# minhtrangvy/distributed_bitcoin_minter

Hardware: AMD Instinct MI355X
Metric: GH/s (SHA-256 "msg nonce" min-search) at 1/2/4/8 MI355X; % of int32 VALU peak (higher is better)
Workload: dtype u32

## Files before the change

### distributed_bitcoin_minter_amd/_lib.py

```python
import ctypes
import os

_HERE = os.path.dirname(os.path.abspath(__file__))
LIB_PATH = os.environ.get("BTCMINER_LIB") or os.path.join(_HERE, "libbtcminer.so")

BM_OK = 0
BM_EINVAL = -1
BM_ENODEV = -2
BM_EHIP = -3
BM_ERCCL = -4
BM_ENOMEM = -5
BM_EINTERNAL = -6
BM_EPEER = -7
BM_ETIMEDOUT = -8
BM_EFULL = -9
BM_MAX_LAUNCH_STATS = 64
BM_MAX_STAT_DEVICES = 16
BM_RCCL_ID_BYTES = 128
BM_ABI_VERSION = 7
BM_DEFAULT_PEER_TIMEOUT_MS = 600_000
BM_COMBINE_AUTO, BM_COMBINE_RCCL, BM_COMBINE_HOST = 0, 1, 2
BM_COMBINED_NONE, BM_COMBINED_RCCL, BM_COMBINED_HOST, BM_COMBINED_LOCAL = 0, 1, 2, 3
COMBINED_NAMES = {0: "none", 1: "rccl", 2: "host", 3: "local"}
U64_MAX = (1 << 64) - 1
# ... 314 lines not shown
                                ctypes.c_size_t, c_u32, c_u32, P(JobVerdict), P(PoolVerifyResult)], ctypes.c_int),
        "bm_jobs_verify_cpu": ([P(PoolJobStruct), ctypes.c_size_t, P(PoolSessionStruct), ctypes.c_size_t, P(JobsSubmit),
                                ctypes.c_size_t, P(JobVerdict), P(PoolVerifyResult)], ctypes.c_int),
        "bm_jobs_verify_gpu": ([vp, P(PoolJobStruct), ctypes.c_size_t, P(PoolSessionStruct), ctypes.c_size_t,
                                P(JobsSubmit), ctypes.c_size_t, P(JobVerdict), P(PoolVerifyResult)], ctypes.c_int),
        "bm_share_set_verify_jobs": ([vp, P(PoolJobStruct), ctypes.c_size_t, P(PoolSessionStruct), ctypes.c_size_t,
                                      P(JobsSubmit), ctypes.c_size_t, P(JobVerdict), P(ShareSetResult)], ctypes.c_int),
        "bm_share_set_create": ([vp, ctypes.c_size_t, P(vp)], ctypes.c_int),
        "bm_share_set_create_cpu": ([ctypes.c_size_t, P(vp)], ctypes.c_int),
        "bm_share_set_destroy": ([vp], None),
        "bm_share_set_clear": ([vp], ctypes.c_int),
        "bm_share_set_count": ([vp, P(c_u64), P(c_u64)], ctypes.c_int),
        "bm_share_set_verify": ([vp, P(JobStruct), P(PoolSessionStruct), ctypes.c_size_t, P(PoolSubmit), ctypes.c_size_t,
                                 c_u32, c_u32, P(JobVerdict), P(ShareSetResult)], ctypes.c_int),
        "bm_ledger_create": ([vp, ctypes.c_size_t, P(vp)], ctypes.c_int),
        "bm_ledger_create_cpu": ([ctypes.c_size_t, P(vp)], ctypes.c_int),
        "bm_ledger_destroy": ([vp], None),
        "bm_ledger_clear": ([vp], ctypes.c_int),
        "bm_ledger_rows": ([vp, P(c_u64)], ctypes.c_int),
        "bm_ledger_read": ([vp, ctypes.c_size_t, ctypes.c_size_t, P(LedgerRow)], ctypes.c_int),
        "bm_ledger_drain": ([vp, ctypes.c_size_t, ctypes.c_size_t, P(LedgerRow)], ctypes.c_int),
        "bm_ledger_set_peel": ([vp, c_u32], ctypes.c_int),
        "bm_ledger_verify_jobs": ([vp, vp, P(PoolJobStruct), ctypes.c_size_t, P(PoolSessionStruct), ctypes.c_size_t,
                                   P(c_u32), P(c_u64), P(JobsSubmit), ctypes.c_size_t, P(JobVerdict),
                                   P(LedgerResult)], ctypes.c_int),
        "bm_hash_gpu": ([vp, ctypes.c_char_p, ctypes.c_size_t, P(c_u64), ctypes.c_size_t, P(c_u64)],
                        ctypes.c_int),
        "bm_ctx_set_timing": ([vp, ctypes.c_int], ctypes.c_int),
        "bm_ctx_last_stats": ([vp, P(Stats)], ctypes.c_int),
        "bm_ctx_set_blocks_per_cu": ([vp, ctypes.c_int], ctypes.c_int),
        "bm_ctx_set_max_windows": ([vp, ctypes.c_int], ctypes.c_int),
        "bm_ctx_set_combine": ([vp, ctypes.c_int], ctypes.c_int),
        "bm_ctx_set_task_digits": ([vp, ctypes.c_int], ctypes.c_int),
        "bm_ctx_set_split": ([vp, P(ctypes.c_uint32), ctypes.c_int], ctypes.c_int),
        "bm_ctx_get_split": ([vp, P(ctypes.c_uint32), ctypes.c_int, P(ctypes.c_int)], ctypes.c_int),
        "bm_ctx_set_balance": ([vp, ctypes.c_int], ctypes.c_int),
        "bm_split_range": ([c_u64, c_u64, P(ctypes.c_uint32), ctypes.c_int, P(c_u64), P(c_u64)], ctypes.c_int),
        "bm_plan_segments": ([ctypes.c_char_p, ctypes.c_size_t, c_u64, c_u64, P(Segment), ctypes.c_int,
                              P(ctypes.c_int)], ctypes.c_int),
        "bm_plan_segments_ex": ([ctypes.c_char_p, ctypes.c_size_t, c_u64, c_u64, ctypes.c_int, P(Segment),
                                 ctypes.c_int, P(ctypes.c_int)], ctypes.c_int),
    }
    for name, (args, res) in sigs.items():
        try:
            fn = getattr(lib, name)
        except AttributeError:
            raise OSError(f"{path}: no {name}; rebuild it") from None
        fn.argtypes = args
        fn.restype = res
    if lib.bm_abi_version() != BM_ABI_VERSION:
        raise OSError(f"{path}: ABI version {lib.bm_abi_version()}, expected {BM_ABI_VERSION}; rebuild it")
    return lib


def strerror(status):
    try:
        return load().bm_strerror(status).decode()
    except OSError:
        return f"status {status}"


def check(status, what):
    if status != BM_OK:
        raise BtcMinerError(status, what)


def device_count():
    n = ctypes.c_int(0)
    check(load().bm_device_count(ctypes.byref(n)), "bm_device_count")
    return n.value


def device_pci_bus_id(device: int) -> str:
    buf = ctypes.create_string_buffer(64)
    check(load().bm_device_pci_bus_id(device, buf, len(buf)), "bm_device_pci_bus_id")
    return buf.value.decode()


DEFAULT_MAX_WINDOWS = 64


def plan_segments(msg: bytes, lower: int, upper: int, max_windows: int = DEFAULT_MAX_WINDOWS):
    lib = load()
    n = ctypes.c_int(0)
    f = lib.bm_plan_segments_ex
    check(f(msg, len(msg), lower, upper, max_windows, None, 0, ctypes.byref(n)), "bm_plan_segments")
    arr = (Segment * max(n.value, 1))()
    check(f(msg, len(msg), lower, upper, max_windows, arr, n.value, ctypes.byref(n)), "bm_plan_segments")
    return list(arr[: n.value])


def split_range(lower: int, upper: int, n: int, shares=None):
    lo, hi = (c_u64 * n)(), (c_u64 * n)()
    sh = (ctypes.c_uint32 * n)(*shares) if shares is not None else None
    check(load().bm_split_range(lower, upper, sh, n, lo, hi), "bm_split_range")
    return [(a, b) if a <= b else None for a, b in zip(lo, hi)]


def bits_to_target(nbits: int) -> int:
    if not 0 <= nbits <= U32_MAX:
        raise ValueError(f"bits must be in 0..2^32-1, got {nbits}")
    buf = (ctypes.c_uint8 * 32)()
    if load().bm_header_target_from_bits(nbits, buf) != BM_OK:
        raise ValueError(f"bits {nbits:#010x} is negative or overflows 256 bits")
    return int.from_bytes(bytes(buf), "big")


def roll_versions(base: int, count: int, mask: int = BIP320_MASK):
    for v, what in ((base, "base"), (mask, "mask")):
        if not isinstance(v, int) or isinstance(v, bool) or not 0 <= v <= U32_MAX:
            raise ValueError(f"{what} must be in 0..2^32-1, got {v!r}")
    if not isinstance(count, int) or isinstance(count, bool) or count < 0:
        raise ValueError(f"count must be a non-negative integer, got {count!r}")
    positions = [b for b in range(32) if mask >> b & 1]
    if count > 1 << len(positions):
        raise ValueError(f"mask {mask:#010x} holds {1 << len(positions)} versions, {count} asked for")
    out = []
    for i in range(count):
        v = base & ~mask
        for k, b in enumerate(positions):
            v |= (i >> k & 1) << b
        out.append(v)
    return out


def difficulty_to_target(difficulty) -> int:
    if isinstance(difficulty, bool) or not isinstance(difficulty, (int, float)):
        raise ValueError(f"difficulty must be a number, got {difficulty!r}")
    try:
# ... 722 lines not shown
            hits = [(int.from_bytes(raw[o:o + 32], "big"), int.from_bytes(raw[o + 32:o + 36], "little"))
                    for o in range(0, len(raw), ctypes.sizeof(HeaderHit))]
        return r.count, hits, (int.from_bytes(bytes(r.hash), "big"), r.nonce)

    def header_hash_many(self, header: bytes, nonces):
        header = _header_bytes(header)
        nonces = list(nonces)
        for v in nonces:
            if not 0 <= v <= U32_MAX:
                raise ValueError(f"a nonce must be in 0..2^32-1, got {v!r}")
        n = len(nonces)
        arr = (c_u32 * max(n, 1))(*nonces)
        out = (ctypes.c_uint8 * (32 * max(n, 1)))()
        check(self._lib.bm_header_hash_gpu(self.handle, header, arr, n, out), "bm_header_hash_gpu")
        raw = bytes(out)
        return [int.from_bytes(raw[32 * i:32 * i + 32], "big") for i in range(n)]

    def hash_many(self, msg: bytes, nonces):
        n = len(nonces)
        arr = (c_u64 * max(n, 1))(*nonces)
        out = (c_u64 * max(n, 1))()
        check(self._lib.bm_hash_gpu(self.handle, msg, len(msg), arr, n, out), "bm_hash_gpu")
        return list(out[:n])

    def set_timing(self, on: bool):
        check(self._lib.bm_ctx_set_timing(self.handle, 1 if on else 0), "bm_ctx_set_timing")

    def set_combine(self, mode: int):
        check(self._lib.bm_ctx_set_combine(self.handle, mode), "bm_ctx_set_combine")

    def set_task_digits(self, digits: int):
        check(self._lib.bm_ctx_set_task_digits(self.handle, digits), "bm_ctx_set_task_digits")

    def set_max_windows(self, n: int):
        check(self._lib.bm_ctx_set_max_windows(self.handle, n), "bm_ctx_set_max_windows")

    def set_blocks_per_cu(self, n: int):
        check(self._lib.bm_ctx_set_blocks_per_cu(self.handle, n), "bm_ctx_set_blocks_per_cu")

    def set_split(self, shares):
        shares = list(shares or [])
        arr = (ctypes.c_uint32 * max(len(shares), 1))(*shares)
        check(self._lib.bm_ctx_set_split(self.handle, arr, len(shares)), "bm_ctx_set_split")

    def get_split(self):
        n = ctypes.c_int(0)
        check(self._lib.bm_ctx_get_split(self.handle, None, 0, ctypes.byref(n)), "bm_ctx_get_split")
        arr = (ctypes.c_uint32 * max(n.value, 1))()
        check(self._lib.bm_ctx_get_split(self.handle, arr, n.value, ctypes.byref(n)), "bm_ctx_get_split")
        return list(arr[: n.value])

    def set_balance(self, on: bool):
        check(self._lib.bm_ctx_set_balance(self.handle, 1 if on else 0), "bm_ctx_set_balance")

    def last_stats(self):
        s = Stats()
        check(self._lib.bm_ctx_last_stats(self.handle, ctypes.byref(s)), "bm_ctx_last_stats")
        return s
```

### distributed_bitcoin_minter_amd/csrc/bm_ctx.cpp

```cpp
#include <algorithm>
#include <cerrno>
#include <cstdarg>
#include <cstdio>
#include <cstdlib>
#include <cstring>
#include <system_error>

#include "bm_runtime.hpp"

namespace bm {

void trace(const char* fmt, ...) {
    static const bool on = std::getenv("BTCMINER_TRACE") != nullptr;
    if (!on) return;
    va_list ap;
    va_start(ap, fmt);
    std::fprintf(stderr, "[btcminer] ");
    std::vfprintf(stderr, fmt, ap);
    std::fprintf(stderr, "\n");
    va_end(ap);
}

bool SubmitPool::run(int n, const std::function<void(int)>& f) {
    if (!ensure(n - 1)) return false;
// ... 119 lines not shown
    for (auto& e : d.ev) BM_TRY(new_event(d, e));
    for (auto& s : d.aux) BM_TRY(new_stream(d, s));
    BM_TRY(new_event(d, d.fork, hipEventDisableTiming));
    for (auto& e : d.join) BM_TRY(new_event(d, e, hipEventDisableTiming));
    for (auto& e : d.bal) BM_TRY(new_event(d, e));
    for (auto& e : d.ag) BM_TRY(new_event(d, e));
    BM_TRY(new_event(d, d.own_done, hipEventDisableTiming));
    BM_TRY(ensure_counters(d, kMinCounterStrips));
    return grow(d, d.d_part, d.part_cap, kMinPartials);
}

void destroy_device(DeviceCtx& d) {
    if (d.id < 0) return;
    (void)hipSetDevice(d.id);
    for (hipStream_t s : d.streams) (void)hipStreamSynchronize(s);
    if (d.comm) (void)ncclCommAbort(d.comm);
    d.comm = nullptr;
    for (hipEvent_t e : d.events) (void)hipEventDestroy(e);
    for (const auto& m : d.owned) (void)(m.second ? hipHostFree(m.first) : hipFree(m.first));
    for (hipStream_t s : d.streams) (void)hipStreamDestroy(s);
}

void read_env(bm_ctx* ctx) {
    if (const char* e = std::getenv("BTCMINER_STREAMS")) {
        const int v = std::atoi(e);
        if (v >= 1 && v <= kMaxStreams) ctx->streams = v;
    }
    if (const char* e = std::getenv("BTCMINER_TAIL")) {
        char* end = nullptr;
        errno = 0;
        const unsigned long long v = std::strtoull(e, &end, 10);
        if (end != e && *end == '\0' && errno == 0 && v <= kMaxTailNonces) ctx->tail_nonces = v;
    }
    if (const char* e = std::getenv("BTCMINER_PADC")) ctx->padc = std::strcmp(e, "0") != 0;
    if (const char* e = std::getenv("BTCMINER_HEADER_GROUP")) {
        const int v = std::atoi(e);
        if (v == 1 || v == 2 || v == 4) ctx->header_group = v;
    }
    if (const char* e = std::getenv("BTCMINER_CHUNK")) {
        char* end = nullptr;
        errno = 0;
        const unsigned long long v = std::strtoull(e, &end, 10);
        if (end != e && *end == '\0' && errno == 0 && v >= 10 && v <= 100000) ctx->lane_chunk = v;
    }
}

int create_ctx(const int* devices, int n, int nslots, bm_ctx** out) {
    int count = 0;
    if (hipGetDeviceCount(&count) != hipSuccess || count < 1) return BM_ENODEV;
    for (int i = 0; i < n; ++i)
        if (devices[i] < 0 || devices[i] >= count) return BM_ENODEV;
    bm_ctx* ctx = new (std::nothrow) bm_ctx();
    if (!ctx) return BM_ENOMEM;
    std::memset(&ctx->stats, 0, sizeof ctx->stats);
    std::memset(&ctx->tstats, 0, sizeof ctx->tstats);
    record_rccl(ctx, false);
    read_env(ctx);
    DeviceGuard guard;
    ctx->devs.resize(n);
    for (int i = 0; i < n; ++i) {
        int rc = init_device(ctx->devs[i], devices[i], nslots);
        if (rc != BM_OK) {
            for (auto& d : ctx->devs) destroy_device(d);
            delete ctx;
            return rc;
        }
// ... 265 lines not shown
}

int bm_ctx_set_test_rccl_fault(bm_ctx_t* ctx, int where) {
    if (!ctx || where < 0 || where > 3) return BM_EINVAL;
    ctx->test_rccl_fault = where;
    return BM_OK;
}

int bm_ctx_set_timing(bm_ctx_t* ctx, int enable) {
    if (!ctx) return BM_EINVAL;
    ctx->timing = enable != 0;
    return BM_OK;
}

int bm_ctx_set_blocks_per_cu(bm_ctx_t* ctx, int blocks_per_cu) {
    if (!ctx || blocks_per_cu < 0 || blocks_per_cu > 32) return BM_EINVAL;
    ctx->blocks_per_cu = blocks_per_cu;
    return BM_OK;
}

int bm_ctx_set_combine(bm_ctx_t* ctx, int mode) {
    if (!ctx || mode < BM_COMBINE_AUTO || mode > BM_COMBINE_HOST) return BM_EINVAL;
    if (ctx->rank_ctx && mode != BM_COMBINE_AUTO) return BM_EINVAL;
    ctx->combine = mode;
    return BM_OK;
}

int bm_ctx_set_task_digits(bm_ctx_t* ctx, int digits) {
    if (!ctx || digits < 0 || digits > bm::kMaxInnerDigits) return BM_EINVAL;
    ctx->task_digits = digits;
    return BM_OK;
}

int bm_ctx_set_max_windows(bm_ctx_t* ctx, int max_windows) {
    if (!ctx || max_windows < 0) return BM_EINVAL;
    ctx->max_windows = max_windows;
    return BM_OK;
}

int bm_ctx_set_split(bm_ctx_t* ctx, const uint32_t* shares, int n) {
    if (!ctx || n < 0 || (n > 0 && !shares)) return BM_EINVAL;
    if (n == 0) {
        ctx->shares.clear();
        return BM_OK;
    }
    const int slots = ctx->rank_ctx ? ctx->world : (int)ctx->devs.size();
    if (n != slots) return BM_EINVAL;
    for (int i = 0; i < n; ++i)
        if (shares[i] == 0) return BM_EINVAL;
    ctx->shares.assign(shares, shares + n);
    return BM_OK;
}

int bm_ctx_get_split(const bm_ctx_t* ctx, uint32_t* shares, int cap, int* n) {
    if (!ctx || !n || cap < 0 || (cap > 0 && !shares)) return BM_EINVAL;
    *n = (int)ctx->shares.size();
    for (int i = 0; i < cap && i < *n; ++i) shares[i] = ctx->shares[(size_t)i];
    return BM_OK;
}

int bm_ctx_set_balance(bm_ctx_t* ctx, int enable) {
    if (!ctx || (ctx->rank_ctx && ctx->world > 1 && enable)) return BM_EINVAL;
    ctx->balance = enable != 0;
    return BM_OK;
}

// ... 34 lines not shown
```

### distributed_bitcoin_minter_amd/csrc/bm_plan.cpp

```cpp
#include "bm_plan.hpp"

#include <algorithm>
#include <cstring>

#include "bm_sha256.hpp"

namespace bm {

const uint64_t kPow10[20] = {1ull,
                             10ull,
                             100ull,
                             1000ull,
                             10000ull,
                             100000ull,
                             1000000ull,
                             10000000ull,
                             100000000ull,
                             1000000000ull,
                             10000000000ull,
                             100000000000ull,
                             1000000000000ull,
                             10000000000000ull,
                             100000000000000ull,
                             1000000000000000ull,
// ... 135 lines not shown

std::vector<Piece> slot_pieces(uint64_t lower, uint64_t upper, int n, const std::vector<uint32_t>& shares) {
    const Piece empty{1, 0};
    if (n < 1) return {};
    if (shares.size() != (size_t)n || lower > upper) {
        std::vector<Piece> out = split_range(lower, upper, n);
        out.resize((size_t)n, empty);
        return out;
    }
    std::vector<Piece> out((size_t)n, empty);
    unsigned __int128 total = 0;
    for (int i = 0; i < n; ++i) total += shares[(size_t)i];
    const unsigned __int128 count = (unsigned __int128)(upper - lower) + 1;
    unsigned __int128 prefix = 0, b0 = 0;
    for (int i = 0; i < n; ++i) {
        prefix += shares[(size_t)i];
        const unsigned __int128 b1 = (i == n - 1) ? count : count * prefix / total;
        if (b1 > b0) out[(size_t)i] = Piece{lower + (uint64_t)b0, lower + (uint64_t)(b1 - 1)};
        b0 = b1;
    }
    return out;
}

LaunchGeometry launch_geometry(uint64_t tasks, uint64_t task_nonces, uint64_t lane_chunk, uint64_t resident,
                               uint32_t block) {
    const uint64_t m_max = std::max<uint64_t>(1, lane_chunk / task_nonces);
    const uint64_t m = std::max<uint64_t>(1, std::min<uint64_t>(m_max, tasks / (8 * resident * (uint64_t)block)));
    const uint64_t chunks = (tasks + 64 * m - 1) / (64 * m);
    const uint64_t grid = std::max<uint64_t>(1, std::min<uint64_t>((chunks + 3) / 4, resident));
    const uint64_t k = (chunks + grid * 4 - 1) / (grid * 4);
    return LaunchGeometry{(uint32_t)m, chunks, (uint32_t)grid, k * m};
}

}
```

### distributed_bitcoin_minter_amd/csrc/bm_plan.hpp

```cpp
#pragma once
#include <cstddef>
#include <cstdint>
#include <vector>

#include "btcminer.h"

namespace bm {

extern const uint64_t kPow10[20];

int decimal_digits(uint64_t v);

constexpr int kDefaultMaxWindows = 64;

int plan_segments(const uint8_t* msg, size_t len, uint64_t lower, uint64_t upper,
                  std::vector<bm_segment_t>& segs, int max_windows = kDefaultMaxWindows);

struct Piece {
    uint64_t lo, hi;
};
std::vector<Piece> split_range(uint64_t lower, uint64_t upper, int n);

std::vector<Piece> slot_pieces(uint64_t lower, uint64_t upper, int n, const std::vector<uint32_t>& shares);

struct LaunchGeometry {
    uint32_t chunk_m;
    uint64_t chunks;
    uint32_t grid;
    uint64_t tasks_per_thread;
};
LaunchGeometry launch_geometry(uint64_t tasks, uint64_t task_nonces, uint64_t lane_chunk, uint64_t resident,
                               uint32_t block);

}
```

### distributed_bitcoin_minter_amd/csrc/bm_runtime.hpp

```cpp
#pragma once
#include <hip/hip_runtime_api.h>
#include <rccl/rccl.h>

#include <chrono>
#include <condition_variable>
#include <cstdint>
#include <functional>
#include <memory>
#include <mutex>
#include <new>
#include <thread>
#include <utility>
#include <vector>

#include "bm_common.h"
#include "bm_header.hpp"
#include "bm_header_versions.hpp"
#include "bm_plan.hpp"
#include "btcminer.h"

#ifndef BM_CLOCK_PROBE
#define BM_CLOCK_PROBE 0
#endif

namespace bm {

constexpr int kMaxInnerDigits = 2;
constexpr uint32_t kNoncesPerLaneChunk = 100;
constexpr int kEventPairs = BM_MAX_LAUNCH_STATS;
constexpr int kMaxStreams = 4;
constexpr uint64_t kMaxTailNonces = 1ull << 40;
constexpr size_t kCtrStride = 32;
constexpr int kCtrClockSlot = 16;
constexpr size_t kMinCounterStrips = 256, kMinPartials = 4096;

struct Slot {
    Partial p;
    uint64_t status;
    uint64_t pad;
};
static_assert(sizeof(Slot) == 32, "slot layout");
constexpr size_t kSlotWords = sizeof(Slot) / sizeof(uint64_t);

struct DeviceCtx {
    int id = -1;
    int cus = 0;
    std::vector<std::pair<void*, bool>> owned;
    std::vector<hipEvent_t> events;
    std::vector<hipStream_t> streams;
    hipStream_t stream = nullptr;
    Partial* d_part = nullptr;
    size_t part_cap = 0;
    unsigned long long* d_ctr = nullptr;
    unsigned long long* h_ctr = nullptr;
    size_t ctr_cap = 0, hctr_cap = 0;
    unsigned long long* d_hit = nullptr;
    unsigned long long* h_hit = nullptr;
    unsigned long long* d_hcount = nullptr;
    unsigned long long* h_hcount = nullptr;
    Partial* d_hbuf = nullptr;
// ... 14 lines not shown
    hipEvent_t ev[2 * kEventPairs] = {};
    hipStream_t aux[kMaxStreams - 1] = {};
    hipEvent_t fork = nullptr, join[kMaxStreams - 1] = {};
    hipEvent_t bal[2] = {};
    hipEvent_t ag[2] = {};
    hipEvent_t own_done = nullptr;
    uint64_t piece_nonces = 0;
    std::chrono::steady_clock::time_point submitted{};
    int test_delay_us = 0;
    ncclComm_t comm = nullptr;
    std::vector<std::pair<const void*, int>> occ;
    double wall_clock_hz = 100e6;
};

enum class Kind { Search, Target, Hits, HeaderVersions, HeaderVersionsHits };
struct Mode {
    Kind kind = Kind::Search;
    uint64_t target = 0;
    uint64_t cap = 0;
    bool first_hit() const { return kind == Kind::Target || kind == Kind::HeaderVersions; }
    bool every_hit() const { return kind == Kind::Hits || kind == Kind::HeaderVersionsHits; }
    bool target64() const { return kind == Kind::Target || kind == Kind::Hits; }
};

struct Launch {
    const void* fn;
    union {
        SearchArgs search;
        HeaderVersionsArgs<kMaxVersionSlots> versions;
    } args;
    uint64_t first_nonce;
    uint64_t tasks;
    uint64_t task_nonces;
    bm_launch_stat_t stat;
};

struct JoinJob {
    std::mutex m;
    std::condition_variable cv;
    bool done = false, abandoned = false;
    ncclComm_t comm = nullptr;
    int rc = BM_ERCCL;
    double init_ms = 0.0;
};

inline int hip_status(hipError_t e) { return e == hipSuccess ? BM_OK : BM_EHIP; }

#define BM_HIP(call)                                     \
    do {                                                 \
        hipError_t e_ = (call);                          \
        if (e_ != hipSuccess) return bm::hip_status(e_); \
    } while (0)
#define BM_TRY(call)   \
    do {                                                                   \
        const int rc_ = (call);                                            \
        if (rc_ != BM_OK) return rc_;                                      \
    } while (0)

void trace(const char* fmt, ...);

class SubmitPool {
   public:
    SubmitPool() = default;
    SubmitPool(const SubmitPool&) = delete;
    SubmitPool& operator=(const SubmitPool&) = delete;
    ~SubmitPool() { stop(); }
// ... 14 lines not shown
    bool quit_ = false;
};

struct DeviceGuard {
    int prev = -1;
    DeviceGuard() {
        if (hipGetDevice(&prev) != hipSuccess) prev = -1;
    }
    ~DeviceGuard() {
        if (prev >= 0) (void)hipSetDevice(prev);
    }
};

template <class F>
int guarded(F&& f) noexcept {
    try {
        return f();
    } catch (const std::bad_alloc&) {
        return BM_ENOMEM;
    } catch (...) {
        return BM_EINTERNAL;
    }
}

}

struct bm_ctx {
    std::vector<bm::DeviceCtx> devs;
    bool timing = false;
    int blocks_per_cu = 0;
    int max_windows = bm::kDefaultMaxWindows;
    int combine = BM_COMBINE_AUTO;
    int task_digits = 0;
    uint64_t tail_nonces = 1ull << 24;
    int streams = 2;
    bool nccl_ready = false;
    int rccl_status = 0;
    int rank = 0, world = 1;
    bool rank_ctx = false;
    bool joined = false;
    int group_status = 0;
    int peer_timeout_ms = BM_DEFAULT_PEER_TIMEOUT_MS;
    double rccl_init_ms = 0.0;
    int fault_after = -1;
    int test_rccl_fault = 0;
    uint64_t lane_chunk = bm::kNoncesPerLaneChunk;
    std::vector<uint32_t> shares;
    bool balance = false;
    int header_group = bm::kMaxVersionSlots;
    bool padc = true;
    std::shared_ptr<bm::JoinJob> pending_join;
    std::thread pending_worker;
    bm_stats_t stats;
    bm_target_stats_t tstats;
    bm::SubmitPool submit;
};

namespace bm {

int grow_bytes(DeviceCtx& d, void** p, size_t* cap, size_t n, size_t elem, bool pinned, int oom_status);
template <class T>
int grow(DeviceCtx& d, T*& p, size_t& cap, size_t n, size_t elem = sizeof(T), bool pinned = false,
         int oom_status = BM_EHIP) {
    return grow_bytes(d, reinterpret_cast<void**>(&p), &cap, n, elem, pinned, oom_status);
}
int ensure_counters(DeviceCtx& d, size_t strips);
// ... 12 lines not shown
```

### distributed_bitcoin_minter_amd/csrc/bm_search.cpp

```cpp
#include <algorithm>
#include <atomic>
#include <cmath>
#include <cstdio>
#include <cstring>

#include "bm_header_versions_hits.hpp"
#include "bm_job.hpp"
#include "bm_runtime.hpp"

namespace bm {

const void* g_header_hash = nullptr;

namespace {

constexpr int kSearchRows = 3 + kMaxPadPrefixBlocks;
const void* g_search[kSearchRows][64];
const void* g_target[2][64];
const void* g_hits[2][64];
const void* g_header_versions[kMaxVersionSlots + 1];
const void* g_header_versions_hits[kMaxVersionSlots + 1];

constexpr uint64_t kBalanceMinNonces = 1ull << 30;
constexpr double kShareScale = 65536.0;
// ... 40 lines not shown
}

int pad_fold_k(const bm_segment_t& s) {
    if (!s.pad_block || s.nbv != 1 || s.p < 55) return -1;
    const uint32_t bits = s.pad_w[15];
    if (bits % 8 != 0 || bits / 8 < (uint32_t)s.p + 1 || (bits / 8 - s.p - 1) % 64 != 0) return -1;
    const uint32_t k = (bits / 8 - s.p - 1) / 64;
    if (k > (uint32_t)kMaxPadPrefixBlocks) return -1;
    uint32_t w[64];
    for (int i = 0; i < 16; ++i) w[i] = s.pad_w[i];
    host::expand(w);
    const KW64 kw = pad_kw_const(s.p, (int)k);
    for (int t = 0; t < 64; ++t)
        if (kK256[t] + w[t] != kw.v[t]) return -1;
    if (k == 0)
        for (int q = 0; q < 8; ++q)
            if (s.mid[q] != kIV256[q]) return -1;
    return (int)k;
}

struct DevicePlan {
    DeviceCtx& d;
    const int di;
    const Piece piece;
    std::vector<Launch>& list;
    uint32_t off = 0;
    void push(Launch& L) {
        L.stat.device = di;
        off += L.stat.grid;
        list.push_back(L);
    }
};

int size_launch(bm_ctx* ctx, DevicePlan& dp, Kind kind, const bm_segment_t& s) {
    const int fk = (ctx->padc && kind == Kind::Search) ? pad_fold_k(s) : -1;
    const void* fn = fk >= 0 ? g_search[2 + fk][s.p] : nullptr;
    const bool padc = fn != nullptr;
    if (!fn) fn = (kind == Kind::Target ? g_target : kind == Kind::Hits ? g_hits : g_search)[s.nbv - 1][s.p];
    if (!fn) return BM_EINTERNAL;
    int ms = std::max(1, std::min(s.max_inner, kMaxInnerDigits));
    if (s.p % 4 == 0 && s.p / 4 >= 1 && s.nd >= 2) ms = 2;
    const uint64_t resident = resident_blocks(ctx, dp.d, fn);
    if (ctx->task_digits > 0) {
        ms = std::min(ms, ctx->task_digits);
    } else if (ms > 1) {
        const uint64_t lanes = resident * (uint64_t)kBlock;
        const uint64_t tasks100 = (s.vhi - s.vlo) / 100 + 1;
        if (tasks100 < 2 * lanes) ms = 1;
    }
    const uint64_t S = kPow10[ms];
    const uint64_t t0 = s.vlo / S, t_end = s.vhi / S + 1;
    const LaunchGeometry g = launch_geometry(t_end - t0, S, ctx->lane_chunk, resident, kBlock);

    Launch L;
    std::memset(&L, 0, sizeof L);
    SearchArgs& A = L.args.search;
    std::memcpy(A.mid, s.mid, sizeof A.mid);
    std::memcpy(A.tmpl, s.tmpl, sizeof A.tmpl);
    if (s.pad_block) {
        uint32_t w[64];
        for (int i = 0; i < 16; ++i) w[i] = s.pad_w[i];
        host::expand(w);
        for (int i = 0; i < 64; ++i) A.padkw[i] = kK256[i] + w[i];
    }
    A.vlo = s.vlo;
    A.vhi = s.vhi;
    A.nonce_base = s.nonce_base;
    A.t0 = t0;
    A.t_end = t_end;
    A.chunk_m = g.chunk_m;
    A.S = (uint32_t)S;
    A.ms = (uint32_t)ms;
    A.nd = (uint32_t)s.nd;
    A.part_off = dp.off;
    L.fn = fn;
    L.first_nonce = s.nonce_base + s.vlo;
    L.tasks = t_end - t0;
    L.task_nonces = S;
    L.stat.p = s.p;
    L.stat.nbv = s.nbv;
    L.stat.pad_block = padc ? 2 + fk : s.pad_block;
    L.stat.digits = s.digits;
    L.stat.inner_digits = ms;
    L.stat.nonces = s.vhi - s.vlo + 1;
    L.stat.grid = g.grid;
    L.stat.tasks_per_thread = (uint32_t)g.tasks_per_thread;
    dp.push(L);
    return BM_OK;
}

int size_header_launch(bm_ctx* ctx, DevicePlan& dp, Kind kind, const HeaderVersionsArgs<kMaxVersionSlots>& base,
                       int m) {
    const void* fn = (kind == Kind::HeaderVersionsHits ? g_header_versions_hits : g_header_versions)[m];
    if (!fn) return BM_EINTERNAL;
    const uint32_t lo = (uint32_t)dp.piece.lo, hi = (uint32_t)dp.piece.hi;
    Launch L;
    std::memset(&L, 0, sizeof L);
    HeaderVersionsArgs<kMaxVersionSlots>& A = L.args.versions;
    A = base;
    A.lo = lo;
    A.hi = hi;
    A.t0 = lo >> kHeaderTaskBits;
    A.ntask = (hi >> kHeaderTaskBits) - A.t0 + 1;
    const LaunchGeometry g = launch_geometry(A.ntask, kHeaderTaskNonces, ctx->lane_chunk,
                                             resident_blocks(ctx, dp.d, fn), kBlock);
    A.chunk_m = g.chunk_m;
    A.part_off = dp.off;
    L.fn = fn;
    L.first_nonce = lo;
    L.tasks = A.ntask;
    L.task_nonces = (uint64_t)kHeaderTaskNonces * (uint64_t)m;
// ... 21 lines not shown
    for (int di = 0; di < ndev; ++di)
        ctx->devs[di].piece_nonces = pieces[di].lo <= pieces[di].hi ? pieces[di].hi - pieces[di].lo + 1 : 0;
    return pieces;
}

int ensure_buffers(DeviceCtx& d, const Mode& mode, const std::vector<Launch>& launches) {
    size_t parts = 0;
    for (const Launch& L : launches) parts += L.stat.grid;
    BM_TRY(grow(d, d.d_part, d.part_cap, std::max(parts, kMinPartials)));
    BM_TRY(ensure_counters(d, launches.size()));
    if (!mode.every_hit()) return BM_OK;
    return grow(d, d.d_hbuf, d.hbuf_cap, std::max<size_t>(mode.cap, 1), sizeof(Partial), false, BM_ENOMEM);
}

template <class PerDevice>
int plan_devices(bm_ctx* ctx, const Mode& mode, uint64_t lower, uint64_t upper,
                 std::vector<std::vector<Launch>>& launches, PerDevice&& per_device) {
    const std::vector<Piece> pieces = plan_pieces(ctx, lower, upper);
    for (size_t di = 0; di < pieces.size(); ++di) {
        if (pieces[di].lo > pieces[di].hi) continue;
        DevicePlan dp{ctx->devs[di], (int)di, pieces[di], launches[di]};
        BM_HIP(hipSetDevice(dp.d.id));
        BM_TRY(per_device(dp));
        BM_TRY(ensure_buffers(dp.d, mode, launches[di]));
    }
    return BM_OK;
}

int plan_decimal(bm_ctx* ctx, const Mode& mode, const uint8_t* msg, size_t len, uint64_t lower, uint64_t upper,
                 std::vector<std::vector<Launch>>& launches) {
    return plan_devices(ctx, mode, lower, upper, launches, [&](DevicePlan& dp) -> int {
        std::vector<bm_segment_t> segs;
        BM_TRY(plan_segments(msg, len, dp.piece.lo, dp.piece.hi, segs, ctx->max_windows));
        if (ctx->streams > 1 && ctx->tail_nonces > 0 && !segs.empty()) {
            size_t big = 0;
            for (size_t i = 1; i < segs.size(); ++i)
                if (segs[i].vhi - segs[i].vlo > segs[big].vhi - segs[big].vlo) big = i;
            bm_segment_t& b = segs[big];
            if ((b.vhi - b.vlo) / 8 >= ctx->tail_nonces) {
                bm_segment_t t = b;
                t.vlo = b.vhi - ctx->tail_nonces + 1;
                b.vhi = t.vlo - 1;
                segs.push_back(t);
            }
        }
        for (const bm_segment_t& seg : segs) BM_TRY(size_launch(ctx, dp, mode.kind, seg));
        return BM_OK;
    });
}

int plan_versions(bm_ctx* ctx, const Mode& mode, const uint8_t* header, const uint32_t* versions, size_t nver,
                  const uint8_t* target, uint32_t lo, uint32_t hi, std::vector<std::vector<Launch>>& launches) {
    uint8_t sizes[BM_MAX_HEADER_VERSIONS];
    const int ngroups = host::versions_groups(nver, ctx->header_group, sizes);
    std::vector<HeaderVersionsArgs<kMaxVersionSlots>> groups((size_t)ngroups);
    size_t at = 0;
    for (int g = 0; g < ngroups; ++g) {
        std::memset(&groups[g], 0, sizeof groups[g]);
        if (!host::header_versions_precompute(header, versions, at, sizes[g], groups[g])) return BM_EINTERNAL;
        for (int i = 0; i < 8; ++i) groups[g].tgt[i] = host::load_be32(target + 4 * i);
        at += sizes[g];
    }
    BM_TRY(plan_devices(ctx, mode, lo, hi, launches, [&](DevicePlan& dp) -> int {
        for (int g = 0; g < ngroups; ++g) BM_TRY(size_header_launch(ctx, dp, mode.kind, groups[g], sizes[g]));
        return BM_OK;
    }));
    ctx->stats.nonces *= nver;
    return BM_OK;
}

void drain(bm_ctx* ctx) {
    for (auto& d : ctx->devs) {
        if (hipSetDevice(d.id) != hipSuccess) continue;
        for (hipStream_t s : d.streams) (void)hipStreamSynchronize(s);
    }
    (void)hipGetLastError();
}

int enqueue_device(bm_ctx* ctx, int di, const Mode& mode, std::vector<Launch>& launches, uint32_t& first,
                   std::atomic<int>& enqueued) {
    DeviceCtx& d = ctx->devs[di];
    const bool mark = ctx->balance || ctx->timing;
    const size_t strip_bytes = launches.size() * kCtrStride * sizeof(unsigned long long);
    BM_HIP(hipSetDevice(d.id));
    if (d.test_delay_us > 0) std::this_thread::sleep_for(std::chrono::microseconds(d.test_delay_us));
    if (mark) BM_HIP(hipEventRecord(d.bal[0], d.stream));
    d.submitted = std::chrono::steady_clock::now();
    if (!launches.empty()) BM_HIP(hipMemsetAsync(d.d_ctr, 0, strip_bytes, d.stream));
    if (mode.first_hit()) {
        *d.h_hit = ~0ull;
        BM_HIP(hipMemsetAsync(d.d_hit, 0xFF, sizeof(unsigned long long), d.stream));
    }
    if (mode.every_hit()) {
        *d.h_hcount = 0;
        BM_HIP(hipMemsetAsync(d.d_hcount, 0, sizeof(unsigned long long), d.stream));
    }
    const int ns = std::max(1, std::min<int>(ctx->streams, (int)launches.size()));
    std::vector<uint32_t> order(launches.size());
    for (uint32_t i = 0; i < order.size(); ++i) order[i] = i;
    if (mode.first_hit())
        std::stable_sort(order.begin(), order.end(),
                         [&](uint32_t x, uint32_t y) { return launches[x].first_nonce < launches[y].first_nonce; });
    else if (ns > 1)
        std::stable_sort(order.begin(), order.end(),
                         [&](uint32_t x, uint32_t y) { return launches[x].stat.nonces > launches[y].stat.nonces; });
    if (ns > 1) {
        BM_HIP(hipEventRecord(d.fork, d.stream));
        for (int k = 0; k + 1 < ns; ++k) BM_HIP(hipStreamWaitEvent(d.aux[k], d.fork, 0));
    }
    if (!order.empty()) first = order[0];
    uint32_t nparts = 0;
    for (uint32_t r = 0; r < order.size(); ++r) {
        const uint32_t li = order[r];
        Launch& L = launches[li];
        hipStream_t s = (r % ns) == 0 ? d.stream : d.aux[r % ns - 1];
        if (ctx->fault_after >= 0 && enqueued.fetch_add(1) >= ctx->fault_after) return BM_EINTERNAL;
        const bool timed = ctx->timing && li < (uint32_t)kEventPairs;
        if (timed) BM_HIP(hipEventRecord(d.ev[2 * li], s));
        unsigned long long* ctr = d.d_ctr + kCtrStride * li;
        uint64_t target = mode.target, cap = mode.cap;
        void* params[7] = {&L.args, &d.d_part, &ctr};
        int np = 3;
        if (mode.target64()) params[np++] = &target;
        if (mode.first_hit()) params[np++] = &d.d_hit;
        if (mode.every_hit()) {
            params[np++] = &d.d_hcount;
            params[np++] = &d.d_hbuf;
            params[np++] = &cap;
        }
        BM_HIP(hipLaunchKernel(L.fn, dim3(L.stat.grid), dim3(kBlock), params, 0, s));
        if (timed) BM_HIP(hipEventRecord(d.ev[2 * li + 1], s));
        nparts += L.stat.grid;
    }
    for (int k = 0; k + 1 < ns; ++k) {
        BM_HIP(hipEventRecord(d.join[k], d.aux[k]));
        BM_HIP(hipStreamWaitEvent(d.stream, d.join[k], 0));
    }
    BM_TRY(launch_reduce_partials(d.d_part, nparts, &d.d_slot->p, d.stream));
// ... 13 lines not shown
    if (ctx->fault_after == 0) return BM_EINTERNAL;
    std::atomic<int> enqueued{0};
    ctx->stats.start_threads = 1;
    auto one = [&](int di) {
        return guarded([&] { return enqueue_device(ctx, di, mode, launches[di], first[di], enqueued); });
    };
    if (ndev == 1) return one(0);
    std::vector<int> rc(ndev, BM_OK);
    const std::function<void(int)> job = [&](int di) { rc[di] = one(di); };
    bool pooled = false;
    try {
        pooled = ctx->submit.run(ndev, job);
    } catch (...) {
        pooled = false;
    }
    if (!pooled)
        for (int di = 0; di < ndev; ++di) rc[di] = one(di);
    ctx->stats.start_threads = pooled ? 1 + ctx->submit.threads() : 1;
    for (int r : rc)
        if (r != BM_OK) return r;
    return BM_OK;
}

void stamp_common(bm_ctx* ctx) {
    bm_stats_t& st = ctx->stats;
    st.rccl_version = rccl_version();
    const bool have = ctx->rank_ctx ? ctx->joined && ctx->devs[0].comm != nullptr : ctx->nccl_ready;
    st.rccl_init_ms = have ? ctx->rccl_init_ms : 0.0;
    if (st.start_threads == 0) st.start_threads = 1;
}

void begin_call(bm_ctx* ctx, const Mode& mode) {
    std::memset(&ctx->stats, 0, sizeof ctx->stats);
    if (mode.first_hit()) std::memset(&ctx->tstats, 0, sizeof ctx->tstats);
    record_rccl(ctx, false);
    stamp_common(ctx);
}

int fail_call(bm_ctx* ctx, int rc, int rccl_status = 0) {
    drain(ctx);
    std::memset(&ctx->stats, 0, sizeof ctx->stats);
    record_rccl(ctx, false);
    ctx->stats.rccl_status = rccl_status;
    stamp_common(ctx);
    return rc;
}

std::vector<double> start_offsets(bm_ctx* ctx) {
    const int ndev = (int)ctx->devs.size();
    std::vector<double> start_ms(ndev, 0.0);
    auto t0 = ctx->devs[0].submitted;
    for (const auto& d : ctx->devs) t0 = std::min(t0, d.submitted);
    for (int di = 0; di < ndev; ++di)
        start_ms[di] = std::chrono::duration<double, std::milli>(ctx->devs[di].submitted - t0).count();
    return start_ms;
}

int record_stats(bm_ctx* ctx, std::vector<std::vector<Launch>>& launches, const std::vector<uint32_t>& first,
                 const std::vector<double>& start_ms, std::chrono::steady_clock::time_point t_start) {
    bm_stats_t& st = ctx->stats;
    const int ndev = (int)ctx->devs.size();
    st.devices = (uint32_t)std::min(ndev, BM_MAX_STAT_DEVICES);
    for (int di = 0; di < ndev; ++di) {
        DeviceCtx& d = ctx->devs[di];
        if (di < BM_MAX_STAT_DEVICES) {
            st.dev_nonces[di] = d.piece_nonces;
            if (ctx->timing || ctx->balance) st.dev_start_ms[di] = start_ms[di];
            float ms = 0.f;
            if ((ctx->timing || ctx->balance) && hipSetDevice(d.id) == hipSuccess &&
                hipEventElapsedTime(&ms, d.bal[0], d.bal[1]) == hipSuccess)
                st.dev_span_ms[di] = ms;
        }
        uint32_t li = 0;
        const bool span_ok = ctx->timing && !launches[di].empty() && first[di] < (uint32_t)kEventPairs;
        for (Launch& L : launches[di]) {
            ++st.launches;
            if (ctx->timing && li < (uint32_t)kEventPairs) {
                float ms = 0.f;
                BM_HIP(hipEventElapsedTime(&ms, d.ev[2 * li], d.ev[2 * li + 1]));
                L.stat.ms = ms;
                st.kernel_ms += ms;
                const unsigned long long* c = d.h_ctr + kCtrStride * li + kCtrClockSlot - 1;
                if (BM_CLOCK_PROBE && c[4] > c[2] && c[3] > c[1])
                    L.stat.clock_ghz = (double)(c[3] - c[1]) / ((double)(c[4] - c[2]) / d.wall_clock_hz) / 1e9;
                if (span_ok) {
                    float sp = 0.f;
                    BM_HIP(hipEventElapsedTime(&sp, d.ev[2 * first[di]], d.ev[2 * li + 1]));
                    st.span_ms = std::max(st.span_ms, (double)sp);
                }
            }
            if (st.recorded < BM_MAX_LAUNCH_STATS) st.launch[st.recorded++] = L.stat;
            ++li;
        }
    }
    stamp_common(ctx);
    st.wall_ms = std::chrono::duration<double, std::milli>(std::chrono::steady_clock::now() - t_start).count();
    return BM_OK;
}

uint64_t scan_hit_words(bm_ctx* ctx, const std::vector<std::vector<Launch>>& launches) {
    bm_target_stats_t& ts = ctx->tstats;
    const int ndev = (int)ctx->devs.size();
    uint64_t hit = UINT64_MAX;
    ts.devices = (uint32_t)std::min(ndev, BM_MAX_STAT_DEVICES);
    for (int di = 0; di < ndev; ++di) {
        const DeviceCtx& d = ctx->devs[di];
        if (launches[di].empty()) continue;
        if (hit == UINT64_MAX) hit = *d.h_hit;
        uint64_t disp = 0;
        for (size_t li = 0; li < launches[di].size(); ++li) {
            const Launch& L = launches[di][li];
            const uint64_t tasks = std::min<uint64_t>(d.h_ctr[kCtrStride * li], L.tasks);
            disp += std::min<uint64_t>(tasks * L.task_nonces, L.stat.nonces);
        }
        if (di < BM_MAX_STAT_DEVICES) ts.dev_dispatched[di] = disp;
        ts.nonces_dispatched += disp;
    }
    return hit;
}

struct Call {
    bool empty = false;
    std::vector<std::vector<Launch>> launches;
    std::vector<uint32_t> first;
// ... 379 lines not shown
```

### include/btcminer.h

```cpp
#ifndef BTCMINER_H
#define BTCMINER_H

#include <stddef.h>
#include <stdint.h>

#ifdef __cplusplus
extern "C" {
#endif

#define BM_ABI_VERSION 7

#define BM_OK 0
#define BM_EINVAL (-1)
#define BM_ENODEV (-2)
#define BM_EHIP (-3)
#define BM_ERCCL (-4)
#define BM_ENOMEM (-5)
#define BM_EINTERNAL (-6)
#define BM_EPEER (-7)
#define BM_ETIMEDOUT (-8)
#define BM_EFULL (-9)

#define BM_MAX_MSG_LEN (1u << 20)

// ... 314 lines not shown
    uint64_t dev_nonces[BM_MAX_STAT_DEVICES];
    double dev_span_ms[BM_MAX_STAT_DEVICES];
    int32_t rccl_nranks;
    int32_t rccl_rank;
    int32_t dev_rccl_rank[BM_MAX_STAT_DEVICES];
    int32_t dev_rccl_device[BM_MAX_STAT_DEVICES];
    int32_t rccl_version;
    int32_t start_threads;
    double rccl_init_ms;
    double rccl_allgather_ms;
    double combine_ms;
    double dev_allgather_ms[BM_MAX_STAT_DEVICES];
    double dev_start_ms[BM_MAX_STAT_DEVICES];
    bm_launch_stat_t launch[BM_MAX_LAUNCH_STATS];
} bm_stats_t;

int bm_ctx_set_timing(bm_ctx_t* ctx, int enable);
int bm_ctx_last_stats(const bm_ctx_t* ctx, bm_stats_t* out);

typedef struct bm_target_stats {
    uint64_t nonces_dispatched;
    uint64_t dev_dispatched[BM_MAX_STAT_DEVICES];
    uint32_t devices;
    uint32_t reserved;
} bm_target_stats_t;
int bm_ctx_last_target_stats(const bm_ctx_t* ctx, bm_target_stats_t* out);

int bm_ctx_set_blocks_per_cu(bm_ctx_t* ctx, int blocks_per_cu);

int bm_ctx_set_max_windows(bm_ctx_t* ctx, int max_windows);

int bm_ctx_set_task_digits(bm_ctx_t* ctx, int digits);

#define BM_COMBINE_AUTO 0
#define BM_COMBINE_RCCL 1
#define BM_COMBINE_HOST 2
int bm_ctx_set_combine(bm_ctx_t* ctx, int mode);

#define BM_MAX_SLOTS 1024
int bm_ctx_set_split(bm_ctx_t* ctx, const uint32_t* shares, int n);
int bm_ctx_get_split(const bm_ctx_t* ctx, uint32_t* shares, int cap, int* n);
int bm_ctx_set_balance(bm_ctx_t* ctx, int enable);
int bm_split_range(uint64_t lower, uint64_t upper, const uint32_t* shares, int n, uint64_t* lo, uint64_t* hi);


#define BM_MAX_REDUCE (1u << 24)
int bm_reduce_gpu(bm_ctx_t* ctx, const bm_result_t* parts, size_t n, bm_result_t* out);

int bm_ctx_set_test_fault(bm_ctx_t* ctx, int launches);

int bm_ctx_set_test_rccl_fault(bm_ctx_t* ctx, int where);

int bm_ctx_set_test_start_delay(bm_ctx_t* ctx, int device, int delay_us);


typedef struct bm_segment {
    int32_t p;
    int32_t nbv;
    int32_t pad_block;
    int32_t digits;
    int32_t nd;
    int32_t max_inner;
    uint64_t vlo, vhi;
    uint64_t nonce_base;
    uint32_t mid[8];
    uint32_t tmpl[32];
// ... 13 lines not shown
```

Before: 53.69.

## Split largest segment into a 3-digit bulk piece plus 2-digit remainder

Raises the maximum inner-digit count to 3 and carves a 1000-aligned bulk region (14/16 of the largest segment by default) that runs with 3-digit tasks, so more nonces share per-task precomputation of the message schedule. The unaligned head and the remainder run as separate launches with fewer digits, and the remainder is reordered to run on a stream right after the bulk launch so the two overlap. It also adds APIs for configuring the split and for reading launch start nonces. The cost is more launches and larger per-task work, which can hurt load balance on small ranges; a minimum size threshold guards against that.

After: 53.66 (median of 2 runs). About the same (-0.1%).

```diff
diff --git a/distributed_bitcoin_minter_amd/_lib.py b/distributed_bitcoin_minter_amd/_lib.py
--- a/distributed_bitcoin_minter_amd/_lib.py
+++ b/distributed_bitcoin_minter_amd/_lib.py
@@ -370,6 +370,10 @@
         "bm_ctx_set_max_windows": ([vp, ctypes.c_int], ctypes.c_int),
         "bm_ctx_set_combine": ([vp, ctypes.c_int], ctypes.c_int),
         "bm_ctx_set_task_digits": ([vp, ctypes.c_int], ctypes.c_int),
+        "bm_ctx_set_bulk": ([vp, ctypes.c_int, c_u64], ctypes.c_int),
+        "bm_plan_bulk_split": ([c_u64, c_u64, ctypes.c_int, c_u64, P(c_u64), P(c_u64), P(ctypes.c_int),
+                                P(ctypes.c_int)], ctypes.c_int),
+        "bm_ctx_last_launch_starts": ([vp, P(c_u64), ctypes.c_int, P(ctypes.c_int)], ctypes.c_int),
         "bm_ctx_set_split": ([vp, P(ctypes.c_uint32), ctypes.c_int], ctypes.c_int),
         "bm_ctx_get_split": ([vp, P(ctypes.c_uint32), ctypes.c_int, P(ctypes.c_int)], ctypes.c_int),
         "bm_ctx_set_balance": ([vp, ctypes.c_int], ctypes.c_int),
@@ -433,6 +437,12 @@
     sh = (ctypes.c_uint32 * n)(*shares) if shares is not None else None
     check(load().bm_split_range(lower, upper, sh, n, lo, hi), "bm_split_range")
     return [(a, b) if a <= b else None for a, b in zip(lo, hi)]
+
+
+def plan_bulk_split(vlo: int, vhi: int, share16: int, min_nonces: int):
+    lo, hi, ms, n = (c_u64 * 3)(), (c_u64 * 3)(), (ctypes.c_int * 3)(), ctypes.c_int(0)
+    check(load().bm_plan_bulk_split(vlo, vhi, share16, min_nonces, lo, hi, ms, ctypes.byref(n)), "bm_plan_bulk_split")
+    return [(lo[i], hi[i], ms[i]) for i in range(n.value)]
 
 
 def bits_to_target(nbits: int) -> int:
@@ -1221,6 +1231,17 @@
     def set_task_digits(self, digits: int):
         check(self._lib.bm_ctx_set_task_digits(self.handle, digits), "bm_ctx_set_task_digits")
 
+    def set_bulk(self, share16: int, min_nonces: int = 0):
+        check(self._lib.bm_ctx_set_bulk(self.handle, share16, min_nonces), "bm_ctx_set_bulk")
+
+    def last_launch_ranges(self):
+        st = self.last_stats()
+        n = ctypes.c_int(0)
+        arr = (c_u64 * max(st.recorded, 1))()
+        check(self._lib.bm_ctx_last_launch_starts(self.handle, arr, st.recorded, ctypes.byref(n)),
+              "bm_ctx_last_launch_starts")
+        return [(arr[i], st.launch[i].nonces) for i in range(min(n.value, st.recorded))]
+
     def set_max_windows(self, n: int):
         check(self._lib.bm_ctx_set_max_windows(self.handle, n), "bm_ctx_set_max_windows")
 
diff --git a/distributed_bitcoin_minter_amd/csrc/bm_ctx.cpp b/distributed_bitcoin_minter_amd/csrc/bm_ctx.cpp
--- a/distributed_bitcoin_minter_amd/csrc/bm_ctx.cpp
+++ b/distributed_bitcoin_minter_amd/csrc/bm_ctx.cpp
@@ -175,6 +175,18 @@
         const unsigned long long v = std::strtoull(e, &end, 10);
         if (end != e && *end == '\0' && errno == 0 && v <= kMaxTailNonces) ctx->tail_nonces = v;
     }
+    if (const char* e = std::getenv("BTCMINER_BULK")) {
+        char* end = nullptr;
+        errno = 0;
+        const unsigned long long v = std::strtoull(e, &end, 10);
+        if (end != e && *end == '\0' && errno == 0 && v <= 16) ctx->bulk_share16 = (uint32_t)v;
+    }
+    if (const char* e = std::getenv("BTCMINER_BULK_MIN")) {
+        char* end = nullptr;
+        errno = 0;
+        const unsigned long long v = std::strtoull(e, &end, 10);
+        if (end != e && *end == '\0' && errno == 0) ctx->bulk_min = v;
+    }
     if (const char* e = std::getenv("BTCMINER_PADC")) ctx->padc = std::strcmp(e, "0") != 0;
     if (const char* e = std::getenv("BTCMINER_HEADER_GROUP")) {
         const int v = std::atoi(e);
@@ -506,6 +518,33 @@
     return BM_OK;
 }
 
+int bm_ctx_set_bulk(bm_ctx_t* ctx, int share16, uint64_t min_nonces) {
+    if (!ctx || share16 < 0 || share16 > 16) return BM_EINVAL;
+    ctx->bulk_share16 = (uint32_t)share16;
+    ctx->bulk_min = min_nonces;
+    return BM_OK;
+}
+
+int bm_plan_bulk_split(uint64_t vlo, uint64_t vhi, int share16, uint64_t min_nonces, uint64_t* lo, uint64_t* hi,
+                       int* ms, int* n) {
+    if (share16 < 0 || share16 > 16 || !lo || !hi || !ms || !n) return BM_EINVAL;
+    const bm::BulkSplit s = bm::split_bulk(vlo, vhi, (uint32_t)share16, min_nonces);
+    *n = s.n;
+    for (int i = 0; i < s.n; ++i) {
+        lo[i] = s.piece[i].vlo;
+        hi[i] = s.piece[i].vhi;
+        ms[i] = s.piece[i].ms;
+    }
+    return BM_OK;
+}
+
+int bm_ctx_last_launch_starts(const bm_ctx_t* ctx, uint64_t* first_nonce, int cap, int* n) {
+    if (!ctx || !n || cap < 0 || (cap > 0 && !first_nonce)) return BM_EINVAL;
+    *n = (int)ctx->launch_first.size();
+    for (int i = 0; i < cap && i < *n; ++i) first_nonce[i] = ctx->launch_first[(size_t)i];
+    return BM_OK;
+}
+
 int bm_ctx_set_max_windows(bm_ctx_t* ctx, int max_windows) {
     if (!ctx || max_windows < 0) return BM_EINVAL;
     ctx->max_windows = max_windows;
diff --git a/distributed_bitcoin_minter_amd/csrc/bm_plan.cpp b/distributed_bitcoin_minter_amd/csrc/bm_plan.cpp
--- a/distributed_bitcoin_minter_amd/csrc/bm_plan.cpp
+++ b/distributed_bitcoin_minter_amd/csrc/bm_plan.cpp
@@ -191,4 +191,23 @@
     return LaunchGeometry{(uint32_t)m, chunks, (uint32_t)grid, k * m};
 }
 
-}
+BulkSplit split_bulk(uint64_t vlo, uint64_t vhi, uint32_t share16, uint64_t min_nonces) {
+    BulkSplit out{};
+    if (share16 == 0 || share16 > 16 || vlo > vhi) return out;
+    const unsigned __int128 count = (unsigned __int128)(vhi - vlo) + 1;
+    if (count < min_nonces) return out;
+    const uint64_t S = kBulkTaskNonces;
+    const uint64_t skip = vlo % S ? S - vlo % S : 0;
+    if (count < (unsigned __int128)skip + S) return out;
+    const uint64_t a = vlo + skip;
+    const unsigned __int128 fit = (count - skip) / S, want = count * share16 / 16 / S;
+    const uint64_t tasks = (uint64_t)std::min(fit, want);
+    if (tasks == 0) return out;
+    const uint64_t end = a + (tasks * S - 1);
+    if (skip) out.piece[out.n++] = BulkPiece{vlo, a - 1, 0};
+    out.piece[out.n++] = BulkPiece{a, end, 3};
+    if (end < vhi) out.piece[out.n++] = BulkPiece{end + 1, vhi, 2};
+    return out;
+}
+
+}
diff --git a/distributed_bitcoin_minter_amd/csrc/bm_plan.hpp b/distributed_bitcoin_minter_amd/csrc/bm_plan.hpp
--- a/distributed_bitcoin_minter_amd/csrc/bm_plan.hpp
+++ b/distributed_bitcoin_minter_amd/csrc/bm_plan.hpp
@@ -32,4 +32,15 @@
 LaunchGeometry launch_geometry(uint64_t tasks, uint64_t task_nonces, uint64_t lane_chunk, uint64_t resident,
                                uint32_t block);
 
+constexpr uint32_t kBulkTaskNonces = 1000;
+struct BulkPiece {
+    uint64_t vlo, vhi;
+    int ms;
+};
+struct BulkSplit {
+    int n;
+    BulkPiece piece[3];
+};
+BulkSplit split_bulk(uint64_t vlo, uint64_t vhi, uint32_t share16, uint64_t min_nonces);
+
 }
diff --git a/distributed_bitcoin_minter_amd/csrc/bm_runtime.hpp b/distributed_bitcoin_minter_amd/csrc/bm_runtime.hpp
--- a/distributed_bitcoin_minter_amd/csrc/bm_runtime.hpp
+++ b/distributed_bitcoin_minter_amd/csrc/bm_runtime.hpp
@@ -25,7 +25,10 @@
 
 namespace bm {
 
-constexpr int kMaxInnerDigits = 2;
+constexpr int kMaxInnerDigits = 3;
+constexpr int kDefaultInnerDigits = 2;
+constexpr uint32_t kDefaultBulkShare16 = 14;
+constexpr uint64_t kBulkMinNonces = 1ull << 30;
 constexpr uint32_t kNoncesPerLaneChunk = 100;
 constexpr int kEventPairs = BM_MAX_LAUNCH_STATS;
 constexpr int kMaxStreams = 4;
@@ -106,6 +109,7 @@
     uint64_t first_nonce;
     uint64_t tasks;
     uint64_t task_nonces;
+    int piece_ms;
     bm_launch_stat_t stat;
 };
 
@@ -186,6 +190,9 @@
     int max_windows = bm::kDefaultMaxWindows;
     int combine = BM_COMBINE_AUTO;
     int task_digits = 0;
+    uint32_t bulk_share16 = bm::kDefaultBulkShare16;
+    uint64_t bulk_min = 0;
+    std::vector<uint64_t> launch_first;
     uint64_t tail_nonces = 1ull << 24;
     int streams = 2;
     bool nccl_ready = false;
diff --git a/distributed_bitcoin_minter_amd/csrc/bm_search.cpp b/distributed_bitcoin_minter_amd/csrc/bm_search.cpp
--- a/distributed_bitcoin_minter_amd/csrc/bm_search.cpp
+++ b/distributed_bitcoin_minter_amd/csrc/bm_search.cpp
@@ -96,16 +96,30 @@
     }
 };
 
-int size_launch(bm_ctx* ctx, DevicePlan& dp, Kind kind, const bm_segment_t& s) {
-    const int fk = (ctx->padc && kind == Kind::Search) ? pad_fold_k(s) : -1;
-    const void* fn = fk >= 0 ? g_search[2 + fk][s.p] : nullptr;
-    const bool padc = fn != nullptr;
-    if (!fn) fn = (kind == Kind::Target ? g_target : kind == Kind::Hits ? g_hits : g_search)[s.nbv - 1][s.p];
+const void* segment_kernel(bm_ctx* ctx, Kind kind, const bm_segment_t& s, int* fk) {
+    *fk = (ctx->padc && kind == Kind::Search) ? pad_fold_k(s) : -1;
+    const void* fn = *fk >= 0 ? g_search[2 + *fk][s.p] : nullptr;
+    if (fn) return fn;
+    *fk = -1;
+    return (kind == Kind::Target ? g_target : kind == Kind::Hits ? g_hits : g_search)[s.nbv - 1][s.p];
+}
+
+bool bulk_capable(Kind kind, const bm_segment_t& s) {
+    return kind == Kind::Search && s.nbv == 1 && s.max_inner >= kMaxInnerDigits;
+}
+
+int size_launch(bm_ctx* ctx, DevicePlan& dp, Kind kind, const bm_segment_t& s, int piece_ms = 0) {
+    int fk = -1;
+    const void* fn = segment_kernel(ctx, kind, s, &fk);
+    const bool padc = fk >= 0;
     if (!fn) return BM_EINTERNAL;
-    int ms = std::max(1, std::min(s.max_inner, kMaxInnerDigits));
+    const bool three = bulk_capable(kind, s) && (piece_ms == kMaxInnerDigits || ctx->task_digits == kMaxInnerDigits);
+    int ms = std::max(1, std::min(s.max_inner, three ? kMaxInnerDigits : kDefaultInnerDigits));
     if (s.p % 4 == 0 && s.p / 4 >= 1 && s.nd >= 2) ms = 2;
     const uint64_t resident = resident_blocks(ctx, dp.d, fn);
-    if (ctx->task_digits > 0) {
+    if (piece_ms > 0) {
+        ms = std::min(ms, piece_ms);
+    } else if (ctx->task_digits > 0) {
         ms = std::min(ms, ctx->task_digits);
     } else if (ms > 1) {
         const uint64_t lanes = resident * (uint64_t)kBlock;
@@ -141,6 +155,7 @@
     L.first_nonce = s.nonce_base + s.vlo;
     L.tasks = t_end - t0;
     L.task_nonces = S;
+    L.piece_ms = piece_ms;
     L.stat.p = s.p;
     L.stat.nbv = s.nbv;
     L.stat.pad_block = padc ? 2 + fk : s.pad_block;
@@ -228,10 +243,10 @@
     return plan_devices(ctx, mode, lower, upper, launches, [&](DevicePlan& dp) -> int {
         std::vector<bm_segment_t> segs;
         BM_TRY(plan_segments(msg, len, dp.piece.lo, dp.piece.hi, segs, ctx->max_windows));
+        size_t big = 0;
+        for (size_t i = 1; i < segs.size(); ++i)
+            if (segs[i].vhi - segs[i].vlo > segs[big].vhi - segs[big].vlo) big = i;
         if (ctx->streams > 1 && ctx->tail_nonces > 0 && !segs.empty()) {
-            size_t big = 0;
-            for (size_t i = 1; i < segs.size(); ++i)
-                if (segs[i].vhi - segs[i].vlo > segs[big].vhi - segs[big].vlo) big = i;
             bm_segment_t& b = segs[big];
             if ((b.vhi - b.vlo) / 8 >= ctx->tail_nonces) {
                 bm_segment_t t = b;
@@ -240,7 +255,31 @@
                 segs.push_back(t);
             }
         }
-        for (const bm_segment_t& seg : segs) BM_TRY(size_launch(ctx, dp, mode.kind, seg));
+        BulkSplit bulk{};
+        if (ctx->streams > 1 && ctx->bulk_share16 > 0 && !segs.empty() && bulk_capable(mode.kind, segs[big]) &&
+            (ctx->task_digits == 0 || ctx->task_digits == kMaxInnerDigits)) {
+            uint64_t least = ctx->bulk_min;
+            if (least == 0) {
+                int fk = -1;
+                const void* fn = segment_kernel(ctx, mode.kind, segs[big], &fk);
+                if (!fn) return BM_EINTERNAL;
+                const uint64_t lanes = resident_blocks(ctx, dp.d, fn) * (uint64_t)kBlock;
+                least = std::max(kBulkMinNonces, 4 * lanes * (uint64_t)kBulkTaskNonces);
+            }
+            bulk = split_bulk(segs[big].vlo, segs[big].vhi, ctx->bulk_share16, least);
+        }
+        for (size_t i = 0; i < segs.size(); ++i) {
+            if (i != big || bulk.n == 0) {
+                BM_TRY(size_launch(ctx, dp, mode.kind, segs[i]));
+                continue;
+            }
+            for (int k = 0; k < bulk.n; ++k) {
+                bm_segment_t piece = segs[i];
+                piece.vlo = bulk.piece[k].vlo;
+                piece.vhi = bulk.piece[k].vhi;
+                BM_TRY(size_launch(ctx, dp, mode.kind, piece, bulk.piece[k].ms));
+            }
+        }
         return BM_OK;
     });
 }
@@ -300,6 +339,18 @@
     else if (ns > 1)
         std::stable_sort(order.begin(), order.end(),
                          [&](uint32_t x, uint32_t y) { return launches[x].stat.nonces > launches[y].stat.nonces; });
+    if (ns > 1 && !mode.first_hit()) {
+        const auto role = [&](int ms) {
+            return std::find_if(order.begin(), order.end(), [&](uint32_t x) { return launches[x].piece_ms == ms; });
+        };
+        const auto b = role(kMaxInnerDigits), s = role(kDefaultInnerDigits);
+        if (b != order.end() && s != order.end() && s != b + 1) {
+            if (s > b)
+                std::rotate(b + 1, s, s + 1);
+            else
+                std::rotate(s, s + 1, b + 1);
+        }
+    }
     if (ns > 1) {
         BM_HIP(hipEventRecord(d.fork, d.stream));
         for (int k = 0; k + 1 < ns; ++k) BM_HIP(hipStreamWaitEvent(d.aux[k], d.fork, 0));
@@ -379,6 +430,7 @@
 
 void begin_call(bm_ctx* ctx, const Mode& mode) {
     std::memset(&ctx->stats, 0, sizeof ctx->stats);
+    ctx->launch_first.clear();
     if (mode.first_hit()) std::memset(&ctx->tstats, 0, sizeof ctx->tstats);
     record_rccl(ctx, false);
     stamp_common(ctx);
@@ -387,6 +439,7 @@
 int fail_call(bm_ctx* ctx, int rc, int rccl_status = 0) {
     drain(ctx);
     std::memset(&ctx->stats, 0, sizeof ctx->stats);
+    ctx->launch_first.clear();
     record_rccl(ctx, false);
     ctx->stats.rccl_status = rccl_status;
     stamp_common(ctx);
@@ -436,7 +489,10 @@
                     st.span_ms = std::max(st.span_ms, (double)sp);
                 }
             }
-            if (st.recorded < BM_MAX_LAUNCH_STATS) st.launch[st.recorded++] = L.stat;
+            if (st.recorded < BM_MAX_LAUNCH_STATS) {
+                st.launch[st.recorded++] = L.stat;
+                ctx->launch_first.push_back(L.first_nonce);
+            }
             ++li;
         }
     }
diff --git a/include/btcminer.h b/include/btcminer.h
--- a/include/btcminer.h
+++ b/include/btcminer.h
@@ -370,6 +370,13 @@
 
 int bm_ctx_set_task_digits(bm_ctx_t* ctx, int digits);
 
+int bm_ctx_set_bulk(bm_ctx_t* ctx, int share16, uint64_t min_nonces);
+
+int bm_plan_bulk_split(uint64_t vlo, uint64_t vhi, int share16, uint64_t min_nonces, uint64_t* lo, uint64_t* hi,
+                       int* ms, int* n);
+
+int bm_ctx_last_launch_starts(const bm_ctx_t* ctx, uint64_t* first_nonce, int cap, int* n);
+
 #define BM_COMBINE_AUTO 0
 #define BM_COMBINE_RCCL 1
 #define BM_COMBINE_HOST 2
```
